# p3achyjr/p3achygo

Measured on AMD Instinct MI355X. Metric: self-play positions/sec at 1/8 MI355X, b12c256btl3 19x19 n=32, higher is better.
Workload: dtype f16

## Files before the change

p3achygo_amd/csrc/conv16.h:

```cpp
#pragma once
#include <type_traits>
#include "conv_core.h"

namespace p3 {

template <class G, int COUT_PASS>
struct Tiling16 {
  using T = Tiling<G, COUT_PASS>;
  static constexpr int CG = T::CG, LG = T::LG;
  static constexpr int MT = 4;
  static constexpr int NT = 2 * T::NT;
  static constexpr int RS = T::RS;
  static_assert(NT >= MT, "A reads are spread over the first MT location groups");
};

template <class G, int COUT_PASS>
__device__ __forceinline__ int tile16_slot0(int lg, int j, bool* valid_tile = nullptr) {
  using T = Tiling16<G, COUT_PASS>;
  int t = lg + (j >> 1) * T::LG;
  const bool ok = t < G::NT_TOTAL;
  if (!ok) t = lg;
  if (valid_tile) *valid_tile = ok;
  const int p = t / G::NT_POS, tt = t - p * G::NT_POS;
  return p * G::PSLOTS + G::PADTOP + tt * 32 + (j & 1);
// ... 239 lines not shown
  const int lane = launder(threadIdx.x & 63);
  const int wid = __builtin_amdgcn_readfirstlane(threadIdx.x >> 6);
  const int lg = wid / T::CG;
  const int n = lane & 15, q = lane >> 4;
  const uint32_t coff = (uint32_t)(((cofs >> 3) + cg_of<G, COUT_PASS>() * 8 + (q >> 1)) * 16);
#pragma unroll
  for (int b = 0; b < NTn / 2; ++b) {
    const int t = lg + b * T::LG;
    const int tv = t < G::NT_TOTAL ? t : lg;
    const int p = tv / G::NT_POS, tt = tv - p * G::NT_POS;
    const int r = tt * 32 + 2 * n + (q & 1);
    int loc;
    const bool ok = row_valid<G::S>(r, loc) && (t < G::NT_TOTAL);
    const uint32_t dst = (uint32_t)((p * G::PSLOTS + G::PADTOP + r) * G::SLOTB) + coff;
#pragma unroll
    for (int ct = 0; ct < 4; ++ct) {
      h4 lo = eo.o[2 * b][ct], hi = eo.o[2 * b + 1][ct];
      if (!PIECES) half_swap(lo, hi);
      if (ok) *(h8*)(smem + dst + ct * 32) = h8{lo[0], lo[1], lo[2], lo[3], hi[0], hi[1], hi[2], hi[3]};
    }
  }
}

template <class G, int COUT_PASS, int NTn>
__device__ __forceinline__ void epilogue_layer16(char* smem, f32x4 (&acc)[4][NTn],
                                                 const float* __restrict__ scale,
                                                 const float* __restrict__ shift) {
  EpiOut16<NTn> eo;
  {
    EpiParams16 ep;
    epi_params16<G, COUT_PASS>(ep, scale, shift, 0);
    epilogue_math16<NTn>(eo, acc, ep);
  }
#pragma unroll
  for (int ct = 0; ct < 4; ++ct)
#pragma unroll
    for (int b = 0; b < NTn / 2; ++b) half_swap(eo.o[2 * b][ct], eo.o[2 * b + 1][ct]);
  lds_barrier();
  epilogue_write16<G, COUT_PASS, NTn, true>(smem, eo, 0);
}

template <int NTn>
struct ResRegs16 {
  static constexpr int NB = NTn / 2;
  h8 rv[NB][4];
  uint32_t base[NB];
  bool ok[NB];
};

template <class G, int COUT_PASS, int NTn>
__device__ __forceinline__ void residual_addr16(ResRegs16<NTn>& rr, int C, int pos0, int npos, int cofs) {
  using T = Tiling16<G, COUT_PASS>;
  const int lane = launder(threadIdx.x & 63);
  const int wid = __builtin_amdgcn_readfirstlane(threadIdx.x >> 6);
  const int lg = wid / T::CG;
  const int n = lane & 15, q = lane >> 4;
  const int cblk = ((cofs + cg_of<G, COUT_PASS>() * 64) >> 3) + (q >> 1);
#pragma unroll
  for (int b = 0; b < NTn / 2; ++b) {
    const int t = lg + b * T::LG;
    const int tv = t < G::NT_TOTAL ? t : lg;
    const int p = tv / G::NT_POS, tt = tv - p * G::NT_POS;
// ... 47 lines not shown
      h4 r0, r1;
      residual_unpack16<NTn>(rr, b, ct, r0, r1);
#pragma unroll
      for (int i = 0; i < 4; ++i) {
        acc[ct][2 * b][i] += (float)r0[i];
        acc[ct][2 * b + 1][i] += (float)r1[i];
      }
    }
}

template <class G, int COUT_PASS, int NTn>
__device__ __forceinline__ void activate_loaded16(EpiOut16<NTn>& A, const ResRegs16<NTn>& xin,
                                                  const float* __restrict__ scale,
                                                  const float* __restrict__ shift, int cofs) {
  const int q = launder(threadIdx.x & 63) >> 4;
  const int c0 = cofs + cg_of<G, COUT_PASS>() * 64 + q * 4;
#pragma unroll
  for (int ct = 0; ct < 4; ++ct) {
    const f32x4 sc = scale_log2e(*(const f32x4*)(scale + c0 + 16 * ct)), sh = scale_log2e(*(const f32x4*)(shift + c0 + 16 * ct));
#pragma unroll
    for (int b = 0; b < NTn / 2; ++b) {
      h4 r0, r1;
      residual_unpack16<NTn>(xin, b, ct, r0, r1);
      bn_mish8_l2(f32x4{(float)r0[0], (float)r0[1], (float)r0[2], (float)r0[3]}, f32x4{(float)r1[0], (float)r1[1], (float)r1[2], (float)r1[3]},
                  sc, sh, sc, sh, A.o[2 * b][ct], A.o[2 * b + 1][ct]);
    }
    __builtin_amdgcn_sched_barrier(0);
  }
}

template <int NTn>
__device__ __forceinline__ void stash16(EpiOut16<NTn>& A, const ResRegs16<NTn>& xin) {
#pragma unroll
  for (int ct = 0; ct < 4; ++ct)
#pragma unroll
    for (int b = 0; b < NTn / 2; ++b) {
      const h8 v = xin.rv[b][ct];
      A.o[2 * b][ct] = h4{v[0], v[1], v[2], v[3]};
      A.o[2 * b + 1][ct] = h4{v[4], v[5], v[6], v[7]};
    }
}
template <class G, int COUT_PASS, int NTn>
__device__ __forceinline__ void activate_stashed16(EpiOut16<NTn>& A, const float* __restrict__ scale,
                                                   const float* __restrict__ shift, int cofs) {
  const int q = launder(threadIdx.x & 63) >> 4;
  const int c0 = cofs + cg_of<G, COUT_PASS>() * 64 + q * 4;
#pragma unroll
  for (int ct = 0; ct < 4; ++ct) {
    const f32x4 sc = scale_log2e(*(const f32x4*)(scale + c0 + 16 * ct)), sh = scale_log2e(*(const f32x4*)(shift + c0 + 16 * ct));
#pragma unroll
    for (int b = 0; b < NTn / 2; ++b) {
      h4 r0 = A.o[2 * b][ct], r1 = A.o[2 * b + 1][ct];
      half_swap(r0, r1);
      bn_mish8_l2(f32x4{(float)r0[0], (float)r0[1], (float)r0[2], (float)r0[3]}, f32x4{(float)r1[0], (float)r1[1], (float)r1[2], (float)r1[3]},
                  sc, sh, sc, sh, A.o[2 * b][ct], A.o[2 * b + 1][ct]);
    }
    __builtin_amdgcn_sched_barrier(0);
  }
}

template <int NTn>
__device__ __forceinline__ void unstash16(EpiOut16<NTn>& A) {
#pragma unroll
  for (int ct = 0; ct < 4; ++ct)
#pragma unroll
    for (int b = 0; b < NTn / 2; ++b) half_swap(A.o[2 * b][ct], A.o[2 * b + 1][ct]);
}

template <class G, int COUT_PASS, int NTn>
__device__ __forceinline__ void epilogue_store16_act(f32x4 (&acc)[4][NTn], const ResRegs16<NTn>& rr,
                                                     _Float16* __restrict__ x, EpiOut16<NTn>& A, bool act,
                                                     const float* __restrict__ scale,
                                                     const float* __restrict__ shift, int cofs) {
  const int q = launder(threadIdx.x & 63) >> 4;
  const int c0 = cofs + cg_of<G, COUT_PASS>() * 64 + q * 4;
  constexpr bool PF = G::NW == 4;
  f32x4 sc = {0, 0, 0, 0}, sh = {0, 0, 0, 0}, nsc = {0, 0, 0, 0}, nsh = {0, 0, 0, 0};
// ... 5 lines not shown
  for (int ct = 0; ct < 4; ++ct) {
    char* xc = (char*)x + (size_t)ct * (2 * kNLoc * 8 * 2);
    if (PF) {
      if (act && ct + 1 < 4) {
        nsc = *(const f32x4*)(scale + c0 + 16 * (ct + 1));
        nsh = *(const f32x4*)(shift + c0 + 16 * (ct + 1));
      }
    } else if (act) {
      sc = *(const f32x4*)(scale + c0 + 16 * ct);
      sh = *(const f32x4*)(shift + c0 + 16 * ct);
    }
    const f32x4 scl = scale_log2e(sc), shl = scale_log2e(sh);
#pragma unroll
    for (int b = 0; b < NTn / 2; ++b) {
      h4 r0, r1;
      residual_unpack16<NTn>(rr, b, ct, r0, r1);
      h4 o0, o1;
#pragma unroll
      for (int i = 0; i < 4; ++i) {
        o0[i] = (_Float16)(acc[ct][2 * b][i] + (float)r0[i]);
        o1[i] = (_Float16)(acc[ct][2 * b + 1][i] + (float)r1[i]);
      }
      if (act) {
        bn_mish8_l2(f32x4{(float)o0[0], (float)o0[1], (float)o0[2], (float)o0[3]}, f32x4{(float)o1[0], (float)o1[1], (float)o1[2], (float)o1[3]},
                    scl, shl, scl, shl, A.o[2 * b][ct], A.o[2 * b + 1][ct]);
      } else {
        A.o[2 * b][ct] = h4{0, 0, 0, 0};
        A.o[2 * b + 1][ct] = h4{0, 0, 0, 0};
      }
      half_swap(o0, o1);
      const h8 piece = {o0[0], o0[1], o0[2], o0[3], o1[0], o1[1], o1[2], o1[3]};
      if (rr.ok[b]) *(h8*)(xc + (uint32_t)(rr.base[b] * 2u)) = piece;
    }
    __builtin_amdgcn_sched_barrier(0);
    if (PF) {
      sc = nsc;
      sh = nsh;
    }
  }
}

template <int NTn>
__device__ __forceinline__ void epilogue_store16_mish(f32x4 (&acc)[4][NTn], const ResRegs16<NTn>& rr,
                                                      _Float16* __restrict__ out) {
#pragma unroll
  for (int ct = 0; ct < 4; ++ct) {
    char* oc = (char*)out + (size_t)ct * (2 * kNLoc * 8 * 2);
// ... 64 lines not shown
```

p3achygo_amd/csrc/conv_core.h:

```cpp
#pragma once
#include <hip/hip_runtime.h>
#include <stdint.h>

namespace p3 {

typedef _Float16 h8 __attribute__((ext_vector_type(8)));
typedef _Float16 h4 __attribute__((ext_vector_type(4)));
typedef _Float16 h2 __attribute__((ext_vector_type(2)));
typedef float f32x16 __attribute__((ext_vector_type(16)));
typedef float f32x4 __attribute__((ext_vector_type(4)));

constexpr int kWG = 512;
constexpr int kNLoc = 361;
constexpr int kBL = 19;
constexpr int kKMS = 4;
constexpr int kRingSlots = 3;
constexpr int kRingDepth = 2;
#ifndef P3_RING_DEPTH4
#define P3_RING_DEPTH4 2
#endif
constexpr int kRingDepth4 = P3_RING_DEPTH4;
constexpr int ring_slot_bytes(int cout_pass, int kms = kKMS) { return kms * cout_pass * 32; }
constexpr int ring_bytes(int cout_pass, int kms = kKMS, int depth = kRingDepth) { return (depth + 1) * ring_slot_bytes(cout_pass, kms); }

// ... 38 lines not shown

typedef float f32x2 __attribute__((ext_vector_type(2)));
__device__ __forceinline__ f32x2 mish_f2(f32x2 x) {
  const f32x2 t = x * 1.4426950408889634f;
  const f32x2 s = f32x2{__builtin_amdgcn_exp2f(t[0]), __builtin_amdgcn_exp2f(t[1])} + 1.0f;
  const f32x2 d = __builtin_elementwise_fma(s, s, f32x2{1.0f, 1.0f});
  const f32x2 r = {__builtin_amdgcn_rcpf(d[0]), __builtin_amdgcn_rcpf(d[1])};
  return __builtin_elementwise_fma(x * -2.0f, r, x);
}

constexpr float kLog2e = 1.4426950408889634f, kLn2 = 0.6931471805599453f;
__device__ __forceinline__ f32x4 scale_log2e(f32x4 v) { return v * kLog2e; }
__device__ __forceinline__ f32x2 mish_t2(f32x2 t) {
  const f32x2 e = {__builtin_amdgcn_exp2f(t[0]), __builtin_amdgcn_exp2f(t[1])};
  const f32x2 d = __builtin_elementwise_fma(e, e + 2.0f, f32x2{2.0f, 2.0f});
  const f32x2 r = {__builtin_amdgcn_rcpf(d[0]), __builtin_amdgcn_rcpf(d[1])};
  return t * __builtin_elementwise_fma(r, f32x2{-2.0f * kLn2, -2.0f * kLn2}, f32x2{kLn2, kLn2});
}
__device__ __forceinline__ h4 bn_mish4_l2(f32x4 v, f32x4 scl, f32x4 shl) {
  const f32x2 a = mish_t2(__builtin_elementwise_fma(f32x2{v[0], v[1]}, f32x2{scl[0], scl[1]}, f32x2{shl[0], shl[1]}));
  const f32x2 b = mish_t2(__builtin_elementwise_fma(f32x2{v[2], v[3]}, f32x2{scl[2], scl[3]}, f32x2{shl[2], shl[3]}));
  return h4{(_Float16)a[0], (_Float16)a[1], (_Float16)b[0], (_Float16)b[1]};
}
__device__ __forceinline__ void bn_mish8_l2(f32x4 v0, f32x4 v1, f32x4 sc0, f32x4 sh0, f32x4 sc1, f32x4 sh1, h4& o0, h4& o1) {
  f32x2 t[4], w[4];
  t[0] = __builtin_elementwise_fma(f32x2{v0[0], v0[1]}, f32x2{sc0[0], sc0[1]}, f32x2{sh0[0], sh0[1]});
  t[1] = __builtin_elementwise_fma(f32x2{v0[2], v0[3]}, f32x2{sc0[2], sc0[3]}, f32x2{sh0[2], sh0[3]});
  t[2] = __builtin_elementwise_fma(f32x2{v1[0], v1[1]}, f32x2{sc1[0], sc1[1]}, f32x2{sh1[0], sh1[1]});
  t[3] = __builtin_elementwise_fma(f32x2{v1[2], v1[3]}, f32x2{sc1[2], sc1[3]}, f32x2{sh1[2], sh1[3]});
  __builtin_amdgcn_sched_barrier(0);
#pragma unroll
  for (int k = 0; k < 4; ++k) w[k] = f32x2{__builtin_amdgcn_exp2f(t[k][0]), __builtin_amdgcn_exp2f(t[k][1])};
  __builtin_amdgcn_sched_barrier(0);
#pragma unroll
  for (int k = 0; k < 4; ++k) w[k] = __builtin_elementwise_fma(w[k], w[k] + 2.0f, f32x2{2.0f, 2.0f});
  __builtin_amdgcn_sched_barrier(0);
#pragma unroll
  for (int k = 0; k < 4; ++k) w[k] = f32x2{__builtin_amdgcn_rcpf(w[k][0]), __builtin_amdgcn_rcpf(w[k][1])};
  __builtin_amdgcn_sched_barrier(0);
#pragma unroll
  for (int k = 0; k < 4; ++k) t[k] = t[k] * __builtin_elementwise_fma(w[k], f32x2{-2.0f * kLn2, -2.0f * kLn2}, f32x2{kLn2, kLn2});
  __builtin_amdgcn_sched_barrier(0);
  o0 = h4{(_Float16)t[0][0], (_Float16)t[0][1], (_Float16)t[1][0], (_Float16)t[1][1]};
  o1 = h4{(_Float16)t[2][0], (_Float16)t[2][1], (_Float16)t[3][0], (_Float16)t[3][1]};
}

template <int RS, int NW = 8, int D = kRingDepth>
struct Ring {
  static constexpr int DEPTH = D, SLOTS = D + 1;
  static constexpr int G = RS / (NW * 1024);
  static constexpr int PIECE = RS / NW;
  static_assert((G == 1 || G == 2) && G * NW * 1024 == RS, "ring slot size");
  const char* gcur;
  const char* gbeg;
  const char* gend;
  uint32_t fill[D + 1];
  uint32_t use[D + 1];
  uint32_t lds_base;
  int tol;
  int extra;
};

constexpr int kXLoads = 12;

template <int N>
__device__ __forceinline__ void rotate_left(uint32_t (&v)[N]) {
  const uint32_t t = v[0];
// ... 549 lines not shown
```

p3achygo_amd/csrc/engine.cpp:

```cpp
#include <hip/hip_runtime.h>
#include <chrono>

#include <atomic>
#include <cmath>
#include <cstdio>
#include <cstdlib>
#include <cstring>
#include <functional>
#include <map>
#include <memory>
#include <unordered_set>
#include <string>
#include <vector>

#include "../../include/p3hip.h"
#include "kernels.h"
#include "slot_state.h"

namespace {

constexpr float kBnEps = 1e-3f;
constexpr int kNLoc = 361;
constexpr size_t kFeatBytes = sizeof(p3hip_features);
static_assert(sizeof(p3hip_features) == 1860, "p3hip_features layout");
// ... 72 lines not shown
    auto st = stand_ins.find(n);
    if (st != stand_ins.end()) return st->second;
    zeros.emplace_back(expect ? expect : 1, 0.0f);
    Tensor t;
    t.dims = {(int)zeros.back().size()};
    t.data = zeros.back().data();
    return stand_ins[n] = t;
  }
  bool is_broadcast(int i) const { return i % bint == bint - 1; }
};

struct Arena {
  std::vector<unsigned char> host;
  bool bad_stream = false;
  size_t add(const void* p, size_t bytes) {
    size_t off = (host.size() + 255) & ~size_t(255);
    host.resize(off + bytes);
    memcpy(host.data() + off, p, bytes);
    return off;
  }
};

void pack_segment(std::vector<_Float16>& dst, const float* W, int taps, int ntaps_pad,
                  int cin_total, int cout_total, int cin0, int CB, int cout0, int CP) {
  for (int tap = 0; tap < ntaps_pad; ++tap)
    for (int q = 0; q < CB / 16; ++q)
      for (int h = 0; h < 2; ++h)
        for (int co = 0; co < CP; ++co)
          for (int e = 0; e < 8; ++e) {
            int ci = cin0 + q * 16 + h * 8 + e, c = cout0 + co;
            float v = 0.0f;
            if (tap < taps && ci < cin_total && c < cout_total)
              v = W[((size_t)tap * cin_total + ci) * cout_total + c];
            dst.push_back((_Float16)v);
          }
}

void pack_segment_3x3(std::vector<_Float16>& dst, const float* W, int cin_total, int cout_total, int CB, int CP) {
  for (int ky = 0; ky < 3; ++ky)
    for (int q32 = 0; q32 < CB / 32; ++q32)
      for (int kx = 0; kx < 3; ++kx)
        for (int q = 2 * q32; q < 2 * q32 + 2; ++q)
          for (int h = 0; h < 2; ++h)
            for (int co = 0; co < CP; ++co)
              for (int e = 0; e < 8; ++e) {
                const int ci = q * 16 + h * 8 + e, tap = ky * 3 + kx;
                float v = 0.0f;
                if (ci < cin_total && co < cout_total) v = W[((size_t)tap * cin_total + ci) * cout_total + co];
                dst.push_back((_Float16)v);
              }
}

void pack_granule(std::vector<_Float16>& dst, const float* W, int cin_total, int cout_total, int tap, int k0, int cout0,
                  const float* scale) {
  for (int j = 0; j < 2; ++j)
    for (int c = 0; c < 2; ++c)
      for (int h = 0; h < 2; ++h)
        for (int n = 0; n < 32; ++n)
          for (int el = 0; el < 8; ++el) {
            const int co = cout0 + 32 * c + n;
            float v = W[((size_t)tap * cin_total + k0 + 16 * j + 8 * h + el) * cout_total + co];
            if (scale) v *= scale[co];
            dst.push_back((_Float16)v);
          }
}

struct FoldedBN { size_t scale_off, shift_off; };

struct LayerPlan {
  int kw, cin, cout;
  bool pre, act, res, dual;
  FoldedBN pre_bn, out_bn;
  int in_buf, out_buf, out2_buf;
  size_t stream_off = 0;
  int nms = 0;
};

struct BlockPlan {
  int kind;
  std::vector<LayerPlan> layers;
  size_t stream_off = 0;
  int nms = 0;
  size_t stream_bytes = 0;
  FoldedBN bn[p3::kMaxBlockLayers];
  size_t stream2_off = 0, stream3_off = 0;
  int nms2 = 0, nms3 = 0;
  size_t dense_bias_off = 0;
  bool first_fused = false, last_fused = false;
  bool dense_fused = false;
  int head_of = -1, tail_of = -1;
  size_t head_bytes = 0, tail_bytes = 0;
};

}

struct p3hip_engine {
  std::string path, err;
  int batch = 0, device = 0;
  uint32_t flags = 0;
  WeightFile wf;
  int n_cu = 256;
  bool c128_wg8 = false;
  bool runs_contiguous = false;
  bool bcast_fuse = true;
  bool blockw = false;
  struct BlockwRun { size_t first; int nblk; size_t stream_off, prm_off; };
  std::vector<BlockwRun> bw_runs;
// ... 69 lines not shown
    return false;
  }
  template <class T>
  const T* dev(size_t off) const { return reinterpret_cast<const T*>(d_arena + off); }
  bool bind() { return check(hipSetDevice(device), "hipSetDevice"); }
};

namespace {

FoldedBN fold_bn(Arena& ar, const WeightFile& wf, const std::string& prefix, size_t n) {
  const Tensor& g = wf.get(prefix + ".gamma", n);
  const Tensor& b = wf.get(prefix + ".beta", n);
  const Tensor& m = wf.get(prefix + ".mean", n);
  const Tensor& v = wf.get(prefix + ".var", n);
  std::vector<float> sc(n), sh(n);
  for (size_t i = 0; i < n; ++i) {
    sc[i] = g.data[i] / std::sqrt(v.data[i] + kBnEps);
    sh[i] = b.data[i] - m.data[i] * sc[i];
  }
  FoldedBN f;
  f.scale_off = ar.add(sc.data(), n * 4);
  f.shift_off = ar.add(sh.data(), n * 4);
  return f;
}

size_t add_stream(Arena& ar, const std::vector<_Float16>& s, int& nms, int cout_pass) {
  const size_t ms = (size_t)cout_pass * 128;
  if (s.size() * 2 % ms != 0) ar.bad_stream = true;
  nms = (int)(s.size() * 2 / ms);
  return ar.add(s.data(), s.size() * 2);
}

bool build_plan(p3hip_engine* e, Arena& ar) {
  const WeightFile& wf = e->wf;
  const int C = wf.C, Cb = wf.Cb;
  const bool fused = (C == 256 && Cb == 128) || (C == 128 && Cb == 64);
  const bool classic = wf.btype == 2 && C == 192 && wf.inner == 2;
  const bool bottleneck_ok = wf.btype == 1 || (wf.btype == 0 && wf.inner >= 1 && wf.inner <= 3);
  const bool layerwise = (C == 384 && Cb == 192 && bottleneck_ok) || classic;
  const bool v_ok = wf.V == 32 || wf.V == 48 || wf.V == 64 || wf.V == 80;
  if (!((fused && bottleneck_ok) || layerwise) || wf.H != 32 || !v_ok) {
    e->err = "unsupported architecture for the HIP engine (need (C, Cb) in {(128,64), (256,128), (384,192)} with "
             "btl (1-3 inner layers) or nbt blocks, or C=192 classic blocks of two convs; H=32, V in {32,48,64,80})";
    return false;
  }
  const int CB = classic ? 64 : (layerwise ? 128 : Cb);
// ... 145 lines not shown
        add_layer(0, 3, C, C, !from_xa, bp.bn[0], true, false, false, bp.bn[1], in0, 1, -1);
        add_layer(1, 3, C, C, false, none, false, true, next_layerwise, next_bn0, 1, 0, 3);
      } else if (wf.btype == 0) {
        add_layer(0, 1, C, Cb, !from_xa, bp.bn[0], true, false, false, bp.bn[1], in0, 1, -1);
        int cur = 1;
        for (int j = 1; j <= wf.inner; ++j) {
          add_layer(j, 3, Cb, Cb, false, none, true, false, false, bp.bn[j + 1], cur, 3 - cur, -1);
          cur = 3 - cur;
        }
        add_layer(wf.inner + 1, 1, Cb, C, false, none, false, true, next_layerwise, next_bn0, cur, 0, 3);
      } else {
        add_layer(0, 1, C, Cb, !from_xa, bp.bn[0], false, false, true, bp.bn[1], in0, 1, 2);
        add_layer(1, 3, Cb, Cb, false, none, true, false, false, bp.bn[2], 2, 3, -1);
        add_layer(2, 3, Cb, Cb, false, none, false, true, true, bp.bn[3], 3, 1, 2);
        add_layer(3, 3, Cb, Cb, false, none, true, false, false, bp.bn[4], 2, 3, -1);
        add_layer(4, 3, Cb, Cb, false, none, false, true, true, bp.bn[5], 3, 1, 2);
        add_layer(5, 1, Cb, C, false, none, false, true, next_layerwise, next_bn0, 2, 0, 3);
      }
      have_xa = next_layerwise;
    } else {
      bp.kind = wf.btype;
      const int nconv = (wf.btype == 0) ? wf.inner + 2 : 6;
      for (int j = 0; j < nconv; ++j) bp.bn[j] = fold_bn(ar, wf, p + ".bn" + std::to_string(j), j == 0 ? C : Cb);
      std::vector<_Float16> s;
      for (int ip = 0; ip < C / CB; ++ip) pack_segment(s, W(0, 1, C, Cb), 1, 1, C, Cb, ip * CB, CB, 0, CB);
      for (int j = 1; j < nconv - 1; ++j) pack_segment_3x3(s, W(j, 3, Cb, Cb), Cb, Cb, CB, CB);
      for (int cp = 0; cp < C / CB; ++cp) pack_segment(s, W(nconv - 1, 1, Cb, C), 1, 1, Cb, C, 0, CB, cp * CB, CB);
      run_streams.emplace_back(e->blocks.size(), std::move(s));
    }
    e->blocks.push_back(bp);
  }
  flush_run();
  for (auto& f : layout) f();
  e->runs_contiguous = true;
  if (e->blockw) {
    const int L = wf.inner;
    const float kLog2e = 1.4426950408889634f;
    for (size_t bi = 0; bi < e->blocks.size();) {
      if (e->blocks[bi].kind != 0) { ++bi; continue; }
      size_t n = 1;
      while (bi + n < e->blocks.size() && e->blocks[bi + n].kind == 0) ++n;
      std::vector<_Float16> ws;
      std::vector<float> prm;
      for (size_t b = bi; b < bi + n; ++b) {
        const std::string p = "blocks." + std::to_string(b);
        auto W = [&](int j, int kw, int cin, int cout) {
          return wf.get(p + ".conv" + std::to_string(j) + ".w", (size_t)kw * kw * cin * cout).data;
        };
        const BlockPlan& bp = e->blocks[b];
        auto bn_row = [&](int j, bool shift) {
          const float* v = reinterpret_cast<const float*>(ar.host.data() + (shift ? bp.bn[j].shift_off : bp.bn[j].scale_off));
          std::vector<float> r((size_t)(j == 0 ? C : Cb));
          for (size_t c = 0; c < r.size(); ++c) r[c] = v[c] * kLog2e;
          return r;
        };
        const float* w0 = W(0, 1, C, Cb);
        const std::vector<float> s1 = bn_row(1, false);
        for (int half = 0; half < 2; ++half)
          for (int s0 = 0; s0 < 128; s0 += 64)
            for (int st = 0; st < 4; ++st) pack_granule(ws, w0, C, Cb, 0, 128 * half + 32 * st, s0, s1.data());
        for (int j = 1; j <= L; ++j) {
          const float* wj = W(j, 3, Cb, Cb);
          const std::vector<float> sj = bn_row(j + 1, false);
          for (int ph = 0; ph < 4; ++ph) {
            const int s0 = (ph & 1) * 64, half = ph >> 1;
            for (int ky = 0; ky < 3; ++ky)
              for (int q = 0; q < 2; ++q)
                for (int kx = 0; kx < 3; ++kx) pack_granule(ws, wj, Cb, Cb, ky * 3 + kx, 64 * half + 32 * q, s0, sj.data());
          }
        }
        const float* we = W(L + 1, 1, Cb, C);
        for (int qo = 0; qo < 4; ++qo)
          for (int c = 0; c < 4; ++c) pack_granule(ws, we, Cb, C, 0, 32 * c, 64 * qo, nullptr);
        for (int sh = 0; sh < 2; ++sh) {
          const std::vector<float> r = bn_row(0, sh == 1);
          prm.insert(prm.end(), r.begin(), r.end());
        }
        for (int j = 1; j <= L + 1; ++j) {
// ... 121 lines not shown
    a.tail_shift[0] = e->dev<float>(bb.bn[0].shift_off);
    if (bb.dense_fused) {
      a.tail_dense = 1;
      a.uout = a.uout2 = e->d_u;
      a.dense_bias[0] = e->dev<float>(bb.dense_bias_off);
      a.dense_scale[0] = e->dev<float>(bb.bn[1].scale_off);
      a.dense_shift[0] = e->dev<float>(bb.bn[1].shift_off);
    }
    a.nms_total += (int)(lb.tail_bytes / ms_bytes);
  }
  {
    static const int stagger_env = getenv("P3HIP_STAGGER") ? atoi(getenv("P3HIP_STAGGER")) : -1;
    const bool long_launch = npos >= 3 * e->n_cu * (e->wf.C == 256 || e->c128_wg8 ? 1 : 2);
    const bool shared = (e->flags & P3HIP_FLAG_SHARED_DEVICE) != 0;
    a.stagger = stagger_env >= 0 ? stagger_env : ((a.head || a.tail) && long_launch && !shared ? 10000 : 0);
    static const bool no_pair_turns = getenv("P3HIP_NO_PAIR_TURNS") != nullptr;
    a.pair_turns = !no_pair_turns && e->wf.C == 128 && !e->c128_wg8 && npos >= 4 * e->n_cu;
  }
  for (int b = 0; b < count; ++b) {
    const BlockPlan& bp = e->blocks[first + b];
    a.nms_total += (int)(bp.stream_bytes / ms_bytes);
    for (int j = 0; j < p3::kMaxBlockLayers; ++j) {
      a.blk[b].scale[j] = e->dev<float>(bp.bn[j].scale_off);
      a.blk[b].shift[j] = e->dev<float>(bp.bn[j].shift_off);
    }
  }
  return a;
}

int joined_launch(p3hip_engine* e, size_t first, int npos, p3::BlockArgs* out) {
  static const bool no_join = getenv("P3HIP_NO_JOIN") != nullptr || getenv("P3HIP_NO_FUSE") != nullptr;
  if (no_join || !e->runs_contiguous) return 0;
  std::vector<std::pair<size_t, int>> runs;
  size_t bi = first;
  int nb = 0;
  while (bi < e->blocks.size() && (int)runs.size() < p3::kMaxRuns) {
    const int kind = e->blocks[bi].kind;
    if (kind != 0) break;
    int n = 1;
    while (bi + n < e->blocks.size() && e->blocks[bi + n].kind == kind) ++n;
    if (n > p3::kMaxFuse || nb + n > p3::kMaxLaunchBlocks) break;
    runs.emplace_back(bi, n);
    nb += n;
    bi += n;
    if (bi + 1 < e->blocks.size() && e->blocks[bi].kind == 3 && e->blocks[bi].first_fused && e->blocks[bi].last_fused &&
        e->blocks[bi].dense_fused && e->blocks[bi + 1].kind == 0) ++bi;
    else break;
// ... 3 lines not shown
  p3::BlockArgs a = block_args(e, runs[0].first, runs[0].second, npos);
  a.nruns = (int)runs.size();
  a.nms_total = 0;
  a.tail = 0;
  a.tail_dense = 1;
  const bool closed = !a.head && !(e->blocks[runs.back().first + runs.back().second - 1].tail_of >= 0);
  _Float16* other = closed ? e->d_t : e->d_u;
  a.zin2 = e->d_u;
  a.uout = other;
  a.zin = other;
  a.uout2 = e->d_u;
  const size_t ms_bytes = (size_t)p3::block_macro_step_bytes(e->wf.C, e->c128_wg8);
  int k = 0;
  for (size_t r = 0; r < runs.size(); ++r) {
    a.run_nblk[r] = runs[r].second;
    const BlockPlan& fb = e->blocks[runs[r].first];
    const BlockPlan& lb = e->blocks[runs[r].first + runs[r].second - 1];
    if (fb.head_of >= 0) a.nms_total += (int)(fb.head_bytes / ms_bytes);
    for (int b = 0; b < runs[r].second; ++b, ++k) {
      const BlockPlan& bp = e->blocks[runs[r].first + b];
      a.nms_total += (int)(bp.stream_bytes / ms_bytes);
      for (int j = 0; j < p3::kMaxBlockLayers; ++j) {
        a.blk[k].scale[j] = e->dev<float>(bp.bn[j].scale_off);
        a.blk[k].shift[j] = e->dev<float>(bp.bn[j].shift_off);
      }
    }
    if (r + 1 < runs.size() || lb.tail_of >= 0) {
      const BlockPlan& bb = e->blocks[lb.tail_of];
      a.nms_total += (int)(lb.tail_bytes / ms_bytes);
      a.tail_scale[r] = e->dev<float>(bb.bn[0].scale_off);
      a.tail_shift[r] = e->dev<float>(bb.bn[0].shift_off);
      a.dense_bias[r] = e->dev<float>(bb.dense_bias_off);
      a.dense_scale[r] = e->dev<float>(bb.bn[1].scale_off);
      a.dense_shift[r] = e->dev<float>(bb.bn[1].shift_off);
      if (r + 1 == runs.size()) a.tail = 1;
    }
  }
  for (size_t r = 0; r + 1 < runs.size(); ++r) {
    const BlockPlan& lb = e->blocks[runs[r].first + runs[r].second - 1];
    const BlockPlan& nf = e->blocks[runs[r + 1].first];
    if (lb.stream_off + lb.stream_bytes + lb.tail_bytes + nf.head_bytes != nf.stream_off) return 0;
  }
  *out = a;
  return (int)(last_run_end - first);
}

int fused_run(const p3hip_engine* e, size_t first) {
// ... 701 lines not shown
```

p3achygo_amd/csrc/kernels.h:

```cpp
#pragma once
#include <hip/hip_runtime.h>
#include <stdint.h>

namespace p3 {

constexpr int kOffMoveLogits = 0;
constexpr int kOffMoveProbs = 362;
constexpr int kOffValueProbs = 724;
constexpr int kOffScoreProbs = 726;
constexpr int kOffOptProbs = 1526;
constexpr int kOffErr2 = 1888;
constexpr int kResultFloats = 1889;
constexpr int kOffOptLogits = 1889;
constexpr int kOffOutcomeLogits = 2251;
constexpr int kOffScoreLogits = 2253;
constexpr int kOffOwnership = 3053;
constexpr int kOffGamma = 3414;
constexpr int kOutStride = 3416;

constexpr int kMaxBlockLayers = 8;

constexpr int kMaxFuse = 6;
constexpr int kMaxRuns = 4, kMaxLaunchBlocks = 12;
struct BlockParams {
  const float* scale[kMaxBlockLayers];
  const float* shift[kMaxBlockLayers];
};
struct BlockArgs {
  _Float16* x;
  _Float16* t;
  int npos;
  int nblk;
  const void* wstream;
  int nms_total;
  BlockParams blk[kMaxLaunchBlocks];
  int nruns;
  int run_nblk[kMaxRuns];
  int head, tail;
  const _Float16* zin;
  const _Float16* zin2;
  _Float16* tout;
  const float* tail_scale[kMaxRuns];
  const float* tail_shift[kMaxRuns];
// ... 131 lines not shown
```

p3achygo_amd/csrc/kernels.hip:

```cpp
#include "kernels.h"

#include <hip/hip_runtime.h>

#include <atomic>

#include "conv_core.h"
#include "conv16.h"

namespace p3 {

constexpr int kTtStride = 784;
constexpr int kTtChannels = 128;
constexpr uint32_t kTtBytes = kTtChannels * kTtStride;

struct GeoTt {
  static constexpr int NW = 8, KMS = kKMS, RD = kRingDepth;
  static constexpr int NPOS = 1, CB = 384, NCH = 48, SLOTB = kTtStride, PAD = 0, S = 1, NROWS = 128,
                       NT_POS = 4, PADTOP = 0, PSLOTS = 128, ACT_BYTES = 128 * kTtStride, NT_TOTAL = 4;
};

template <int C>
__device__ __forceinline__ void bdense_passes(Ring<16384>& ring, char* smem, const float* p_bias, const float* p_scale,
                                              const float* p_shift, _Float16* __restrict__ u, int pos, int half, int nch) {
  constexpr int CH = kTtChannels;
// ... 52 lines not shown
  } while (0)
#define P3_SPAN(k)                                                                        \
  do {                                                                                    \
    if (a.spans && blockIdx.x < kSpanWgs && threadIdx.x == 0 && (k) < 8) {                \
      a.spans[blockIdx.x * kSpanSlots + (k)] = __builtin_amdgcn_s_memtime();              \
      a.spans[blockIdx.x * kSpanSlots + 8 + (k)] = __builtin_amdgcn_s_memrealtime();      \
    }                                                                                     \
  } while (0)
#else
#define P3_STAMP(section, k) do {} while (0)
#define P3_SPAN(k) do {} while (0)
#endif

template <int C, int CB, int KIND, int L, int NW = 8, bool BC = false>
__global__ void __launch_bounds__(NW * 64, 2) k_block(BlockArgs a) {
  static_assert(NW == 8 || (NW == 4 && CB == 64), "4-wave workgroups: one 64-channel position each");
  constexpr int NPOS = NW == 8 ? 128 / CB : 1;
  using G = Geo<NPOS, CB, 3, NW, NW == 8 ? kKMS : 2, NW == 8 ? kRingDepth : kRingDepth4>;
  using T = Tiling16<G, CB>;
  constexpr int NT = T::NT;
  extern __shared__ __attribute__((aligned(16))) char smem[];
  constexpr uint32_t kRingOff = G::ACT_BYTES;
  static_assert(C / CB == 2, "two input slices / two output passes");

  P3_SPAN(0);
  act_zero<G>(smem);
  if (BC && a.stagger > 0) {
    const int key = (blockIdx.x >> 3) & 7;
    const unsigned long long until = __builtin_amdgcn_s_memtime() + (unsigned long long)key * a.stagger;
    while (__builtin_amdgcn_s_memtime() < until) __builtin_amdgcn_s_sleep(16);
  }
  Ring<T::RS, NW, G::RD> ring;
  ring_init(ring, smem, a.wstream, a.nms_total, kRingOff);
  lds_barrier();
  P3_SPAN(1);

  int npos_done = 0;
  for (int pos0 = blockIdx.x * NPOS; pos0 < a.npos; pos0 += gridDim.x * NPOS, ++npos_done) {
    EpiOut16<NT> A1;
    if (NW == 4 && a.pair_turns) {
      if ((blockIdx.x >= gridDim.x / 2) != (bool)(npos_done & 1)) __builtin_amdgcn_s_setprio(1);
      else __builtin_amdgcn_s_setprio(0);
    }
    const int nruns = BC ? a.nruns : 1;
    const bool launch_tail = BC && a.tail;
    int blk0 = 0;
// ... 62 lines not shown
        epilogue_write16<G, CB, NT>(smem, A0, 0);
      }
      P3_STAMP(6, 13);
    }
#pragma unroll 1
    for (int blk = 0; blk < nblk; ++blk) {
      const BlockParams& bp = a.blk[blk0 + blk];
      const bool from_hbm = blk == 0 && !head;
      const bool last = blk + 1 == nblk;
      f32x4 acc[4][NT];
      P3_STAMP(blk, 0);
      if (from_hbm) {
        ResRegs16<NT> xin;
        EpiOut16<NT> A0;
        residual_addr16<G, CB, NT>(xin, C, pos0, a.npos, 0);
        residual_load16<NT>(xin, a.x);
        activate_loaded16<G, CB, NT>(A0, xin, bp.scale[0], bp.shift[0], 0);
        residual_addr16<G, CB, NT>(xin, C, pos0, a.npos, CB);
        residual_load16<NT>(xin, a.x);
        stash16<NT>(A1, xin);
        epilogue_write16<G, CB, NT>(smem, A0, 0);
      }
      ring_note_inflight(ring, from_hbm ? (npos_done == 0 ? 24 : (launch_tail ? (a.tail_dense ? 24 : 36) : 48)) : 24);
      acc16_zero<NT>(acc);
      P3_STAMP(blk, 1);
      conv_segment16<G, CB, 1, 1>(ring, smem, acc);
      P3_STAMP(blk, 2);
      if (from_hbm) activate_stashed16<G, CB, NT>(A1, bp.scale[0], bp.shift[0], CB);
      lds_barrier();
      epilogue_write16<G, CB, NT>(smem, A1, 0);
      P3_STAMP(blk, 3);
      conv_segment16<G, CB, 1, 1>(ring, smem, acc);
      P3_STAMP(blk, 4);
      if (KIND == 0) {
#pragma unroll
        for (int j = 1; j <= L; ++j) {
          epilogue_layer16<G, CB, NT>(smem, acc, bp.scale[j], bp.shift[j]);
          acc16_zero<NT>(acc);
          P3_STAMP(blk, 3 + 2 * j);
          conv_segment16_3x3<G, CB>(ring, smem, acc);
          P3_STAMP(blk, 4 + 2 * j);
        }
        epilogue_layer16<G, CB, NT>(smem, acc, bp.scale[L + 1], bp.shift[L + 1]);
      } else {
        ResRegs16<NT> tr;
        residual_addr16<G, CB, NT>(tr, CB, pos0, a.npos, 0);
        epilogue_store16<false, NT>(acc, tr, a.t);
        epilogue_layer16<G, CB, NT>(smem, acc, bp.scale[1], bp.shift[1]);
#pragma unroll
        for (int r = 0; r < 2; ++r) {
          acc16_zero<NT>(acc);
          conv_segment16_3x3<G, CB>(ring, smem, acc);
          epilogue_layer16<G, CB, NT>(smem, acc, bp.scale[2 + 2 * r], bp.shift[2 + 2 * r]);
          acc16_zero<NT>(acc);
          conv_segment16_3x3<G, CB>(ring, smem, acc);
          residual_addr16<G, CB, NT>(tr, CB, pos0, a.npos, 0);
          residual_load16<NT>(tr, a.t);
          residual_add16<NT>(acc, tr);
          if (r == 0) epilogue_store16<false, NT>(acc, tr, a.t);
          epilogue_layer16<G, CB, NT>(smem, acc, bp.scale[3 + 2 * r], bp.shift[3 + 2 * r]);
        }
      }
      P3_STAMP(blk, 11);
      const bool act_next = !last || tail;
      const float* nsc = last ? (tail ? a.tail_scale[run] : bp.scale[0]) : a.blk[blk0 + blk + 1].scale[0];
      const float* nsh = last ? (tail ? a.tail_shift[run] : bp.shift[0]) : a.blk[blk0 + blk + 1].shift[0];
// ... 1352 lines not shown
```

Baseline: 226,300.

## Fold block batch-norm scale into conv weights and shift into accumulator init

For bottleneck blocks, the BN scale (with log2e and ln2 factors) is multiplied into the packed f16 conv weights on the host. The per-channel shift is preloaded into the accumulators before each conv, so the epilogue only evaluates the mish nonlinearity and skips a per-element FMA and the scale/shift loads. It also replaces the f16-to-f32 convert plus FMA in the residual activation paths with v_fma_mix_f32 inline asm. Folding scale into f16 weights can change rounding and overflow behaviour, and a compile flag keeps the unfolded path available.

```diff
diff --git a/p3achygo_amd/csrc/conv16.h b/p3achygo_amd/csrc/conv16.h
--- a/p3achygo_amd/csrc/conv16.h
+++ b/p3achygo_amd/csrc/conv16.h
@@ -285,12 +285,60 @@
   }
 }
 
-template <class G, int COUT_PASS, int NTn>
+struct AccInit16 { f32x4 sh[4]; };
+
+template <class G, int COUT_PASS>
+__device__ __forceinline__ void acc_init_load16(AccInit16& ai, const float* __restrict__ shl) {
+  const int q = launder(threadIdx.x & 63) >> 4;
+  const int c0 = cg_of<G, COUT_PASS>() * 64 + q * 4;
+#pragma unroll
+  for (int ct = 0; ct < 4; ++ct) ai.sh[ct] = *(const f32x4*)(shl + c0 + 16 * ct);
+}
+
+template <int NTn>
+__device__ __forceinline__ void acc16_init(f32x4 (&acc)[4][NTn], const AccInit16& ai) {
+#pragma unroll
+  for (int ct = 0; ct < 4; ++ct)
+#pragma unroll
+    for (int j = 0; j < NTn; ++j) acc[ct][j] = ai.sh[ct];
+}
+
+template <int NTn>
+__device__ __forceinline__ void epilogue_math16_folded(EpiOut16<NTn>& eo, f32x4 (&acc)[4][NTn]) {
+#ifdef P3_EPI_CHAINS
+#pragma unroll
+  for (int j = 0; j < NTn; ++j) {
+#pragma unroll
+    for (int ct = 0; ct < 4; ++ct) {
+      const f32x2 a = mish_t2s(f32x2{acc[ct][j][0], acc[ct][j][1]}), b = mish_t2s(f32x2{acc[ct][j][2], acc[ct][j][3]});
+      eo.o[j][ct] = h4{(_Float16)a[0], (_Float16)a[1], (_Float16)b[0], (_Float16)b[1]};
+    }
+    __builtin_amdgcn_sched_barrier(0);
+  }
+#else
+#pragma unroll
+  for (int j = 0; j < NTn; ++j) {
+#pragma unroll
+    for (int ct = 0; ct < 4; ct += 2) {
+      f32x2 t[4] = {f32x2{acc[ct][j][0], acc[ct][j][1]}, f32x2{acc[ct][j][2], acc[ct][j][3]},
+                    f32x2{acc[ct + 1][j][0], acc[ct + 1][j][1]}, f32x2{acc[ct + 1][j][2], acc[ct + 1][j][3]}};
+      mish8_t2s(t, eo.o[j][ct], eo.o[j][ct + 1]);
+    }
+  }
+#endif
+}
+
+template <class G, int COUT_PASS, int NTn, bool FOLDED = false, bool NEXT = false>
 __device__ __forceinline__ void epilogue_layer16(char* smem, f32x4 (&acc)[4][NTn],
                                                  const float* __restrict__ scale,
-                                                 const float* __restrict__ shift) {
+                                                 const float* __restrict__ shift,
+                                                 const float* __restrict__ next_shl = nullptr) {
   EpiOut16<NTn> eo;
-  {
+  AccInit16 ai;
+  if constexpr (NEXT) acc_init_load16<G, COUT_PASS>(ai, next_shl);
+  if constexpr (FOLDED) {
+    epilogue_math16_folded<NTn>(eo, acc);
+  } else {
     EpiParams16 ep;
     epi_params16<G, COUT_PASS>(ep, scale, shift, 0);
     epilogue_math16<NTn>(eo, acc, ep);
@@ -301,6 +349,7 @@
     for (int b = 0; b < NTn / 2; ++b) half_swap(eo.o[2 * b][ct], eo.o[2 * b + 1][ct]);
   lds_barrier();
   epilogue_write16<G, COUT_PASS, NTn, true>(smem, eo, 0);
+  if constexpr (NEXT) acc16_init<NTn>(acc, ai);
 }
 
 template <int NTn>
@@ -394,7 +443,7 @@
     for (int b = 0; b < NTn / 2; ++b) {
       h4 r0, r1;
       residual_unpack16<NTn>(xin, b, ct, r0, r1);
-      bn_mish8_l2(f32x4{(float)r0[0], (float)r0[1], (float)r0[2], (float)r0[3]}, f32x4{(float)r1[0], (float)r1[1], (float)r1[2], (float)r1[3]},
+      bn_mish8_l2h(r0, r1,
                   sc, sh, sc, sh, A.o[2 * b][ct], A.o[2 * b + 1][ct]);
     }
     __builtin_amdgcn_sched_barrier(0);
@@ -424,7 +473,7 @@
     for (int b = 0; b < NTn / 2; ++b) {
       h4 r0 = A.o[2 * b][ct], r1 = A.o[2 * b + 1][ct];
       half_swap(r0, r1);
-      bn_mish8_l2(f32x4{(float)r0[0], (float)r0[1], (float)r0[2], (float)r0[3]}, f32x4{(float)r1[0], (float)r1[1], (float)r1[2], (float)r1[3]},
+      bn_mish8_l2h(r0, r1,
                   sc, sh, sc, sh, A.o[2 * b][ct], A.o[2 * b + 1][ct]);
     }
     __builtin_amdgcn_sched_barrier(0);
@@ -476,7 +525,7 @@
         o1[i] = (_Float16)(acc[ct][2 * b + 1][i] + (float)r1[i]);
       }
       if (act) {
-        bn_mish8_l2(f32x4{(float)o0[0], (float)o0[1], (float)o0[2], (float)o0[3]}, f32x4{(float)o1[0], (float)o1[1], (float)o1[2], (float)o1[3]},
+        bn_mish8_l2h(o0, o1,
                     scl, shl, scl, shl, A.o[2 * b][ct], A.o[2 * b + 1][ct]);
       } else {
         A.o[2 * b][ct] = h4{0, 0, 0, 0};
diff --git a/p3achygo_amd/csrc/conv_core.h b/p3achygo_amd/csrc/conv_core.h
--- a/p3achygo_amd/csrc/conv_core.h
+++ b/p3achygo_amd/csrc/conv_core.h
@@ -84,27 +84,77 @@
   const f32x2 b = mish_t2(__builtin_elementwise_fma(f32x2{v[2], v[3]}, f32x2{scl[2], scl[3]}, f32x2{shl[2], shl[3]}));
   return h4{(_Float16)a[0], (_Float16)a[1], (_Float16)b[0], (_Float16)b[1]};
 }
+__device__ __forceinline__ void mish8_t2(f32x2 (&t)[4], h4& o0, h4& o1) {
+  f32x2 w[4];
+#pragma unroll
+  for (int k = 0; k < 4; ++k) w[k] = f32x2{__builtin_amdgcn_exp2f(t[k][0]), __builtin_amdgcn_exp2f(t[k][1])};
+  __builtin_amdgcn_sched_barrier(0);
+#pragma unroll
+  for (int k = 0; k < 4; ++k) w[k] = __builtin_elementwise_fma(w[k], w[k] + 2.0f, f32x2{2.0f, 2.0f});
+  __builtin_amdgcn_sched_barrier(0);
+#pragma unroll
+  for (int k = 0; k < 4; ++k) w[k] = f32x2{__builtin_amdgcn_rcpf(w[k][0]), __builtin_amdgcn_rcpf(w[k][1])};
+  __builtin_amdgcn_sched_barrier(0);
+#pragma unroll
+  for (int k = 0; k < 4; ++k) t[k] = t[k] * __builtin_elementwise_fma(w[k], f32x2{-2.0f * kLn2, -2.0f * kLn2}, f32x2{kLn2, kLn2});
+  __builtin_amdgcn_sched_barrier(0);
+  o0 = h4{(_Float16)t[0][0], (_Float16)t[0][1], (_Float16)t[1][0], (_Float16)t[1][1]};
+  o1 = h4{(_Float16)t[2][0], (_Float16)t[2][1], (_Float16)t[3][0], (_Float16)t[3][1]};
+}
+__device__ __forceinline__ void mish8_t2s(f32x2 (&t)[4], h4& o0, h4& o1) {
+  f32x2 w[4];
+#pragma unroll
+  for (int k = 0; k < 4; ++k) w[k] = f32x2{__builtin_amdgcn_exp2f(t[k][0]), __builtin_amdgcn_exp2f(t[k][1])};
+  __builtin_amdgcn_sched_barrier(0);
+#pragma unroll
+  for (int k = 0; k < 4; ++k)
+    w[k] = __builtin_elementwise_fma(w[k], __builtin_elementwise_fma(w[k], f32x2{0.5f, 0.5f}, f32x2{1.0f, 1.0f}), f32x2{1.0f, 1.0f});
+  __builtin_amdgcn_sched_barrier(0);
+#pragma unroll
+  for (int k = 0; k < 4; ++k) w[k] = f32x2{__builtin_amdgcn_rcpf(w[k][0]), __builtin_amdgcn_rcpf(w[k][1])};
+  __builtin_amdgcn_sched_barrier(0);
+#pragma unroll
+  for (int k = 0; k < 4; ++k) t[k] = __builtin_elementwise_fma(-t[k], w[k], t[k]);
+  __builtin_amdgcn_sched_barrier(0);
+  o0 = h4{(_Float16)t[0][0], (_Float16)t[0][1], (_Float16)t[1][0], (_Float16)t[1][1]};
+  o1 = h4{(_Float16)t[2][0], (_Float16)t[2][1], (_Float16)t[3][0], (_Float16)t[3][1]};
+}
+__device__ __forceinline__ f32x2 mish_t2s(f32x2 t) {
+  const f32x2 e = {__builtin_amdgcn_exp2f(t[0]), __builtin_amdgcn_exp2f(t[1])};
+  const f32x2 d = __builtin_elementwise_fma(e, __builtin_elementwise_fma(e, f32x2{0.5f, 0.5f}, f32x2{1.0f, 1.0f}), f32x2{1.0f, 1.0f});
+  const f32x2 r = {__builtin_amdgcn_rcpf(d[0]), __builtin_amdgcn_rcpf(d[1])};
+  return __builtin_elementwise_fma(-t, r, t);
+}
+
+template <bool HI>
+__device__ __forceinline__ float fma_mix(uint32_t x2, float a, float b) {
+  float r;
+  if constexpr (HI) asm("v_fma_mix_f32 %0, %1, %2, %3 op_sel:[1,0,0] op_sel_hi:[1,0,0]" : "=v"(r) : "v"(x2), "v"(a), "v"(b));
+  else asm("v_fma_mix_f32 %0, %1, %2, %3 op_sel_hi:[1,0,0]" : "=v"(r) : "v"(x2), "v"(a), "v"(b));
+  return r;
+}
+__device__ __forceinline__ void fma_mix4(h4 v, f32x4 s, f32x4 c, f32x2& lo, f32x2& hi) {
+  typedef unsigned int u2 __attribute__((ext_vector_type(2)));
+  const u2 w = __builtin_bit_cast(u2, v);
+  lo = f32x2{fma_mix<false>(w[0], s[0], c[0]), fma_mix<true>(w[0], s[1], c[1])};
+  hi = f32x2{fma_mix<false>(w[1], s[2], c[2]), fma_mix<true>(w[1], s[3], c[3])};
+}
+
 __device__ __forceinline__ void bn_mish8_l2(f32x4 v0, f32x4 v1, f32x4 sc0, f32x4 sh0, f32x4 sc1, f32x4 sh1, h4& o0, h4& o1) {
-  f32x2 t[4], w[4];
+  f32x2 t[4];
   t[0] = __builtin_elementwise_fma(f32x2{v0[0], v0[1]}, f32x2{sc0[0], sc0[1]}, f32x2{sh0[0], sh0[1]});
   t[1] = __builtin_elementwise_fma(f32x2{v0[2], v0[3]}, f32x2{sc0[2], sc0[3]}, f32x2{sh0[2], sh0[3]});
   t[2] = __builtin_elementwise_fma(f32x2{v1[0], v1[1]}, f32x2{sc1[0], sc1[1]}, f32x2{sh1[0], sh1[1]});
   t[3] = __builtin_elementwise_fma(f32x2{v1[2], v1[3]}, f32x2{sc1[2], sc1[3]}, f32x2{sh1[2], sh1[3]});
   __builtin_amdgcn_sched_barrier(0);
-#pragma unroll
-  for (int k = 0; k < 4; ++k) w[k] = f32x2{__builtin_amdgcn_exp2f(t[k][0]), __builtin_amdgcn_exp2f(t[k][1])};
-  __builtin_amdgcn_sched_barrier(0);
-#pragma unroll
-  for (int k = 0; k < 4; ++k) w[k] = __builtin_elementwise_fma(w[k], w[k] + 2.0f, f32x2{2.0f, 2.0f});
-  __builtin_amdgcn_sched_barrier(0);
-#pragma unroll
-  for (int k = 0; k < 4; ++k) w[k] = f32x2{__builtin_amdgcn_rcpf(w[k][0]), __builtin_amdgcn_rcpf(w[k][1])};
-  __builtin_amdgcn_sched_barrier(0);
-#pragma unroll
-  for (int k = 0; k < 4; ++k) t[k] = t[k] * __builtin_elementwise_fma(w[k], f32x2{-2.0f * kLn2, -2.0f * kLn2}, f32x2{kLn2, kLn2});
-  __builtin_amdgcn_sched_barrier(0);
-  o0 = h4{(_Float16)t[0][0], (_Float16)t[0][1], (_Float16)t[1][0], (_Float16)t[1][1]};
-  o1 = h4{(_Float16)t[2][0], (_Float16)t[2][1], (_Float16)t[3][0], (_Float16)t[3][1]};
+  mish8_t2(t, o0, o1);
+}
+__device__ __forceinline__ void bn_mish8_l2h(h4 v0, h4 v1, f32x4 sc0, f32x4 sh0, f32x4 sc1, f32x4 sh1, h4& o0, h4& o1) {
+  f32x2 t[4];
+  fma_mix4(v0, sc0, sh0, t[0], t[1]);
+  fma_mix4(v1, sc1, sh1, t[2], t[3]);
+  __builtin_amdgcn_sched_barrier(0);
+  mish8_t2(t, o0, o1);
 }
 
 template <int RS, int NW = 8, int D = kRingDepth>
diff --git a/p3achygo_amd/csrc/engine.cpp b/p3achygo_amd/csrc/engine.cpp
--- a/p3achygo_amd/csrc/engine.cpp
+++ b/p3achygo_amd/csrc/engine.cpp
@@ -118,7 +118,7 @@
 };
 
 void pack_segment(std::vector<_Float16>& dst, const float* W, int taps, int ntaps_pad,
-                  int cin_total, int cout_total, int cin0, int CB, int cout0, int CP) {
+                  int cin_total, int cout_total, int cin0, int CB, int cout0, int CP, const float* scale = nullptr) {
   for (int tap = 0; tap < ntaps_pad; ++tap)
     for (int q = 0; q < CB / 16; ++q)
       for (int h = 0; h < 2; ++h)
@@ -126,13 +126,16 @@
           for (int e = 0; e < 8; ++e) {
             int ci = cin0 + q * 16 + h * 8 + e, c = cout0 + co;
             float v = 0.0f;
-            if (tap < taps && ci < cin_total && c < cout_total)
+            if (tap < taps && ci < cin_total && c < cout_total) {
               v = W[((size_t)tap * cin_total + ci) * cout_total + c];
+              if (scale) v *= scale[c];
+            }
             dst.push_back((_Float16)v);
           }
 }
 
-void pack_segment_3x3(std::vector<_Float16>& dst, const float* W, int cin_total, int cout_total, int CB, int CP) {
+void pack_segment_3x3(std::vector<_Float16>& dst, const float* W, int cin_total, int cout_total, int CB, int CP,
+                      const float* scale = nullptr) {
   for (int ky = 0; ky < 3; ++ky)
     for (int q32 = 0; q32 < CB / 32; ++q32)
       for (int kx = 0; kx < 3; ++kx)
@@ -142,7 +145,10 @@
               for (int e = 0; e < 8; ++e) {
                 const int ci = q * 16 + h * 8 + e, tap = ky * 3 + kx;
                 float v = 0.0f;
-                if (ci < cin_total && co < cout_total) v = W[((size_t)tap * cin_total + ci) * cout_total + co];
+                if (ci < cin_total && co < cout_total) {
+                  v = W[((size_t)tap * cin_total + ci) * cout_total + co];
+                  if (scale) v *= scale[co];
+                }
                 dst.push_back((_Float16)v);
               }
 }
@@ -179,6 +185,8 @@
   int nms = 0;
   size_t stream_bytes = 0;
   FoldedBN bn[p3::kMaxBlockLayers];
+  bool bn_folded = false;
+  size_t shl_off[p3::kMaxBlockLayers] = {};
   size_t stream2_off = 0, stream3_off = 0;
   int nms2 = 0, nms3 = 0;
   size_t dense_bias_off = 0;
@@ -294,6 +302,14 @@
   f.scale_off = ar.add(sc.data(), n * 4);
   f.shift_off = ar.add(sh.data(), n * 4);
   return f;
+}
+
+std::vector<float> bn_row_log2e(const Arena& ar, const FoldedBN& f, size_t n, bool shift) {
+  const float kLog2e = 1.4426950408889634f;
+  const float* v = reinterpret_cast<const float*>(ar.host.data() + (shift ? f.shift_off : f.scale_off));
+  std::vector<float> r(n);
+  for (size_t c = 0; c < n; ++c) r[c] = v[c] * kLog2e;
+  return r;
 }
 
 size_t add_stream(Arena& ar, const std::vector<_Float16>& s, int& nms, int cout_pass) {
@@ -485,10 +501,25 @@
       bp.kind = wf.btype;
       const int nconv = (wf.btype == 0) ? wf.inner + 2 : 6;
       for (int j = 0; j < nconv; ++j) bp.bn[j] = fold_bn(ar, wf, p + ".bn" + std::to_string(j), j == 0 ? C : Cb);
+      bp.bn_folded = p3::kBlockBnFolded && wf.btype == 0;
+      const float kLn2 = 0.6931471805599453f;
+      std::vector<std::vector<float>> wsc(nconv);
+      if (bp.bn_folded) {
+        for (int j = 1; j < nconv; ++j) {
+          wsc[j - 1] = bn_row_log2e(ar, bp.bn[j], Cb, false);
+          if (j > 1)
+            for (float& v : wsc[j - 1]) v *= kLn2;
+          const std::vector<float> shl = bn_row_log2e(ar, bp.bn[j], Cb, true);
+          bp.shl_off[j] = ar.add(shl.data(), shl.size() * 4);
+        }
+        wsc[nconv - 1].assign((size_t)C, kLn2);
+      }
+      auto fold = [&](int j) { return bp.bn_folded ? wsc[j].data() : nullptr; };
       std::vector<_Float16> s;
-      for (int ip = 0; ip < C / CB; ++ip) pack_segment(s, W(0, 1, C, Cb), 1, 1, C, Cb, ip * CB, CB, 0, CB);
-      for (int j = 1; j < nconv - 1; ++j) pack_segment_3x3(s, W(j, 3, Cb, Cb), Cb, Cb, CB, CB);
-      for (int cp = 0; cp < C / CB; ++cp) pack_segment(s, W(nconv - 1, 1, Cb, C), 1, 1, Cb, C, 0, CB, cp * CB, CB);
+      for (int ip = 0; ip < C / CB; ++ip) pack_segment(s, W(0, 1, C, Cb), 1, 1, C, Cb, ip * CB, CB, 0, CB, fold(0));
+      for (int j = 1; j < nconv - 1; ++j) pack_segment_3x3(s, W(j, 3, Cb, Cb), Cb, Cb, CB, CB, fold(j));
+      for (int cp = 0; cp < C / CB; ++cp)
+        pack_segment(s, W(nconv - 1, 1, Cb, C), 1, 1, Cb, C, 0, CB, cp * CB, CB, fold(nconv - 1));
       run_streams.emplace_back(e->blocks.size(), std::move(s));
     }
     e->blocks.push_back(bp);
@@ -498,7 +529,6 @@
   e->runs_contiguous = true;
   if (e->blockw) {
     const int L = wf.inner;
-    const float kLog2e = 1.4426950408889634f;
     for (size_t bi = 0; bi < e->blocks.size();) {
       if (e->blocks[bi].kind != 0) { ++bi; continue; }
       size_t n = 1;
@@ -511,12 +541,7 @@
           return wf.get(p + ".conv" + std::to_string(j) + ".w", (size_t)kw * kw * cin * cout).data;
         };
         const BlockPlan& bp = e->blocks[b];
-        auto bn_row = [&](int j, bool shift) {
-          const float* v = reinterpret_cast<const float*>(ar.host.data() + (shift ? bp.bn[j].shift_off : bp.bn[j].scale_off));
-          std::vector<float> r((size_t)(j == 0 ? C : Cb));
-          for (size_t c = 0; c < r.size(); ++c) r[c] = v[c] * kLog2e;
-          return r;
-        };
+        auto bn_row = [&](int j, bool shift) { return bn_row_log2e(ar, bp.bn[j], (size_t)(j == 0 ? C : Cb), shift); };
         const float* w0 = W(0, 1, C, Cb);
         const std::vector<float> s1 = bn_row(1, false);
         for (int half = 0; half < 2; ++half)
@@ -684,7 +709,7 @@
     a.nms_total += (int)(bp.stream_bytes / ms_bytes);
     for (int j = 0; j < p3::kMaxBlockLayers; ++j) {
       a.blk[b].scale[j] = e->dev<float>(bp.bn[j].scale_off);
-      a.blk[b].shift[j] = e->dev<float>(bp.bn[j].shift_off);
+      a.blk[b].shift[j] = e->dev<float>(bp.bn_folded && j >= 1 ? bp.shl_off[j] : bp.bn[j].shift_off);
     }
   }
   return a;
@@ -734,7 +759,7 @@
       a.nms_total += (int)(bp.stream_bytes / ms_bytes);
       for (int j = 0; j < p3::kMaxBlockLayers; ++j) {
         a.blk[k].scale[j] = e->dev<float>(bp.bn[j].scale_off);
-        a.blk[k].shift[j] = e->dev<float>(bp.bn[j].shift_off);
+        a.blk[k].shift[j] = e->dev<float>(bp.bn_folded && j >= 1 ? bp.shl_off[j] : bp.bn[j].shift_off);
       }
     }
     if (r + 1 < runs.size() || lb.tail_of >= 0) {
diff --git a/p3achygo_amd/csrc/kernels.h b/p3achygo_amd/csrc/kernels.h
--- a/p3achygo_amd/csrc/kernels.h
+++ b/p3achygo_amd/csrc/kernels.h
@@ -19,6 +19,12 @@
 constexpr int kOutStride = 3416;
 
 constexpr int kMaxBlockLayers = 8;
+
+#ifdef P3_BLOCK_BN_UNFOLDED
+constexpr bool kBlockBnFolded = false;
+#else
+constexpr bool kBlockBnFolded = true;
+#endif
 
 constexpr int kMaxFuse = 6;
 constexpr int kMaxRuns = 4, kMaxLaunchBlocks = 12;
diff --git a/p3achygo_amd/csrc/kernels.hip b/p3achygo_amd/csrc/kernels.hip
--- a/p3achygo_amd/csrc/kernels.hip
+++ b/p3achygo_amd/csrc/kernels.hip
@@ -98,6 +98,7 @@
   extern __shared__ __attribute__((aligned(16))) char smem[];
   constexpr uint32_t kRingOff = G::ACT_BYTES;
   static_assert(C / CB == 2, "two input slices / two output passes");
+  constexpr bool FOLD = kBlockBnFolded && KIND == 0;
 
   P3_SPAN(0);
   act_zero<G>(smem);
@@ -206,7 +207,13 @@
         epilogue_write16<G, CB, NT>(smem, A0, 0);
       }
       ring_note_inflight(ring, from_hbm ? (npos_done == 0 ? 24 : (launch_tail ? (a.tail_dense ? 24 : 36) : 48)) : 24);
-      acc16_zero<NT>(acc);
+      if constexpr (FOLD) {
+        AccInit16 ai;
+        acc_init_load16<G, CB>(ai, bp.shift[1]);
+        acc16_init<NT>(acc, ai);
+      } else {
+        acc16_zero<NT>(acc);
+      }
       P3_STAMP(blk, 1);
       conv_segment16<G, CB, 1, 1>(ring, smem, acc);
       P3_STAMP(blk, 2);
@@ -219,13 +226,17 @@
       if (KIND == 0) {
 #pragma unroll
         for (int j = 1; j <= L; ++j) {
-          epilogue_layer16<G, CB, NT>(smem, acc, bp.scale[j], bp.shift[j]);
-          acc16_zero<NT>(acc);
+          if constexpr (FOLD) {
+            epilogue_layer16<G, CB, NT, true, true>(smem, acc, nullptr, nullptr, bp.shift[j + 1]);
+          } else {
+            epilogue_layer16<G, CB, NT>(smem, acc, bp.scale[j], bp.shift[j]);
+            acc16_zero<NT>(acc);
+          }
           P3_STAMP(blk, 3 + 2 * j);
           conv_segment16_3x3<G, CB>(ring, smem, acc);
           P3_STAMP(blk, 4 + 2 * j);
         }
-        epilogue_layer16<G, CB, NT>(smem, acc, bp.scale[L + 1], bp.shift[L + 1]);
+        epilogue_layer16<G, CB, NT, FOLD>(smem, acc, bp.scale[L + 1], bp.shift[L + 1]);
       } else {
         ResRegs16<NT> tr;
         residual_addr16<G, CB, NT>(tr, CB, pos0, a.npos, 0);
```

Result: faster. 229,800, median of 6 (+1.6%).
